# WPI-MMR/gym_solo

Hardware: AMD Instinct MI355X
Metric: env-steps/s (whole node), 4096 Solo8 envs/GPU, 1/2/4/8 MI355X (higher is better)
Workload: dtype f64

## Files before the change

gym_solo_amd/csrc/solo_step_kernel.h:

```cpp
#pragma once

#include "solo_kernel_params.h"
#include "solo_outputs.h"

#if defined(SOLO_STAMPS) && defined(SOLO_STAMPS_LIGHT)
#define SOLO_STAMP(B, i)                                                                          \
  do {                                                                                            \
    if (((i) == 0 || (i) == 14) && solo::lane_id() == 0)                                          \
      (B).stamps[(size_t)(B).stamp_row * 32 + (i)] = __builtin_amdgcn_s_memrealtime();         \
  } while (0)
#elif defined(SOLO_STAMPS)
#ifdef SOLO_STAMPS_EPILOGUE
#define SOLO_STAMP_ON(i) ((i) == 0 || (i) >= 13)
#define SOLO_STAMP_E(B, i) SOLO_STAMP_AT(B, i)
#else
#define SOLO_STAMP_ON(i) true
#endif
#define SOLO_STAMP(B, i) do { if (SOLO_STAMP_ON(i)) SOLO_STAMP_AT(B, i); } while (0)
#define SOLO_STAMP_AT(B, i)                                                                       \
  do {                                                                                            \
    if (solo::lane_id() == 0) {                                                                   \
      const unsigned long long t_ = __builtin_amdgcn_s_memtime();                                 \
      (B).stamps[(size_t)(B).stamp_row * 32 + (i)] = t_;                                            \
      (B).acc[(i)] += t_ - (B).acc[16];                                                           \
      (B).acc[16] = t_;                                                                           \
    }                                                                                             \
  } while (0)
#else
#define SOLO_STAMP(B, i) do {} while (0)
#endif
#ifndef SOLO_STAMP_E
#define SOLO_STAMP_E(B, i) do {} while (0)
#endif

#ifndef SOLO_PGS_SWEEP_HOOK
#define SOLO_PGS_SWEEP_HOOK(it, pend, lam, v) do {} while (0)
#endif

namespace solo {

template <typename T> struct V3 { T x, y, z; };
template <typename T> __device__ __forceinline__ V3<T> operator+(V3<T> a, V3<T> b) { return {a.x + b.x, a.y + b.y, a.z + b.z}; }
template <typename T> __device__ __forceinline__ V3<T> operator-(V3<T> a, V3<T> b) { return {a.x - b.x, a.y - b.y, a.z - b.z}; }
template <typename T> __device__ __forceinline__ V3<T> operator*(T s, V3<T> a) { return {s * a.x, s * a.y, s * a.z}; }
template <typename T> __device__ __forceinline__ T dot(V3<T> a, V3<T> b) { return a.x * b.x + a.y * b.y + a.z * b.z; }
template <typename T> __device__ __forceinline__ V3<T> cross(V3<T> a, V3<T> b) {
  return {a.y * b.z - a.z * b.y, a.z * b.x - a.x * b.z, a.x * b.y - a.y * b.x};
}
template <typename T> __device__ __forceinline__ V3<T> roty(T c, T s, V3<T> v) {
  return {c * v.x + s * v.z, v.y, c * v.z - s * v.x};
}
template <typename T> __device__ __forceinline__ V3<T> ycross(V3<T> r) { return {r.z, T(0), -r.x}; }
template <typename T> __device__ __forceinline__ V3<T> symmul(const T* I, V3<T> v) {
  return {I[0] * v.x + I[3] * v.y + I[4] * v.z, I[3] * v.x + I[1] * v.y + I[5] * v.z,
          I[4] * v.x + I[5] * v.y + I[2] * v.z};
}
template <typename T> __device__ __forceinline__ void rot_inertia_y(T c, T s, const T* I, T* o) {
  const T cc = c * c, ss = s * s, cs = c * s;
  o[0] = cc * I[0] + T(2) * cs * I[4] + ss * I[2];
  o[1] = I[1];
  o[2] = ss * I[0] - T(2) * cs * I[4] + cc * I[2];
  o[3] = c * I[3] + s * I[5];
  o[4] = cs * (I[2] - I[0]) + (cc - ss) * I[4];
  o[5] = c * I[5] - s * I[3];
}
template <typename T> __device__ __forceinline__ T sum_over_group16(T x) { return wave_sum_group16(x); }
template <typename T> __device__ __forceinline__ V3<T> select(bool p, V3<T> a, V3<T> b) { return {p ? a.x : b.x, p ? a.y : b.y, p ? a.z : b.z}; }
template <typename T> __device__ __forceinline__ T both_halves(T x) { return x + wave_other_half16(x); }
template <typename T> __device__ __forceinline__ V3<T> both_halves(V3<T> v) { return {both_halves(v.x), both_halves(v.y), both_halves(v.z)}; }
template <typename T> __device__ __forceinline__ T from_lower(T x) { return wave_from_lower_half16(x); }
template <typename T> __device__ __forceinline__ V3<T> from_lower(V3<T> v) { return {from_lower(v.x), from_lower(v.y), from_lower(v.z)}; }


}
namespace solo {
#ifndef SOLO_PRIO_SWEEPS_F64
#define SOLO_PRIO_SWEEPS_F64 12
#endif
#ifndef SOLO_QUEUE_SPINS
#define SOLO_QUEUE_SPINS (1 << 22)
#endif
#ifndef SOLO_PRIO_BY_ROWS
#define SOLO_PRIO_BY_ROWS 1
#endif
#ifndef SOLO_PRIO_ROWS_1
#define SOLO_PRIO_ROWS_1 11
#define SOLO_PRIO_ROWS_2 17
#define SOLO_PRIO_ROWS_3 23
#endif
__device__ __forceinline__ int priority_by_rows(int rows) { return rows > SOLO_PRIO_ROWS_3 ? 3 : (rows > SOLO_PRIO_ROWS_2 ? 2 : (rows > SOLO_PRIO_ROWS_1 ? 1 : 0)); }
template <typename T> constexpr int kPrioSweeps = sizeof(T) == 4 ? 8 : SOLO_PRIO_SWEEPS_F64;
#ifndef SOLO_F64_WAVES
#define SOLO_F64_WAVES 4
#endif
template <typename T> constexpr int kRowBlockReals = sizeof(T) == 4 ? 64 * 8 + 64 * 8 : (SOLO_F64_WAVES >= 4 ? 800 : 896);
#ifndef SOLO_W4_PIPELINED_BUILD
#define SOLO_W4_PIPELINED_BUILD 0
#endif
#ifndef SOLO_W4_HYBRID_BUILD
#define SOLO_W4_HYBRID_BUILD 1
#endif
constexpr int kLegSlots = 26;

template <typename T> struct RowView {
  int type, body;
  const T* geo;
};
template <typename T> struct StepTables {
  const LegConst<T>* legc;
  const int32_t* rowtype;
  const T (*rowgeo)[4];
  __device__ __forceinline__ RowView<T> row(int lane) const {
    const int tb = rowtype[lane];
    return {tb & 15, (tb >> 4) & 15, rowgeo[(tb >> 8) & 255]};
  }
};

constexpr unsigned long long kPhaseLanes[3] = {0xc003c003c003c003ull,
                                               0x0924092409240924ull,
                                               0x36d836d836d836d8ull};

template <typename T, bool kResid, bool kFromLds>
__device__ __forceinline__ int pgs_solve_cpp(const ColumnBank<T>& A, T& v, T& lamv, T& cand, T& dl, unsigned long long& pend, T& lo, T& hi,
                                             T tol_rel, int lane, T mu, bool is_tan1, bool is_tangent, unsigned long long ph0,
                                             unsigned long long ph1, unsigned long long ph2, int iters, T diag, T resid_thr, int& n_changed) {
  using R = Real<T>;
  int it = 0;
#pragma unroll 1
  for (; it < iters && pend != 0ull; ++it) {
    const T lam_sweep_start = lamv;
    bool normals_moved = false;
#pragma unroll
    for (int phase = 0; phase < 3; ++phase) {
      const unsigned long long phase_lanes = phase == 0 ? ph0 : (phase == 1 ? ph1 : ph2);
      if (phase == 2 && normals_moved) {
        T n1, n2;
        if constexpr (ColumnBank<T>::kCompact) { n1 = wave_slot_below<1>(lamv); n2 = wave_slot_below<2>(lamv); }
        else { n1 = wave_lane_below<1>(lamv); n2 = wave_lane_below<2>(lamv); }
        const T lim = mu * (is_tan1 ? n1 : n2);
        lo = is_tangent ? -lim : lo;
        hi = is_tangent ? lim : hi;
        cand = R::clamp(v, lo, hi);
        dl = cand - lamv;
        pend = wave_ballot(R::abs(dl) > R::abs(lamv) * tol_rel);
      }
      if ((pend & phase_lanes) == 0ull) continue;
      if (phase == 1) normals_moved = true;
#pragma unroll
      for (int bank = 0; bank < (kFromLds ? 1 : ColumnBank<T>::kBanks); ++bank) {
        unsigned long long window = kFromLds ? phase_lanes : (phase_lanes & ColumnBank<T>::bank_lanes(bank));
#pragma unroll 1
        while ((pend & window) != 0ull) {
          const int r = __builtin_ctzll(pend & window);
          window &= ~((2ull << r) - 1ull);
          const T col = kFromLds ? A.column(r) : A.get(bank, r);
          const T delta = wave_readlane(dl, r);
          v = R::fma(col, delta, v);
          lamv = (lane == r) ? cand : lamv;
          cand = R::clamp(v, lo, hi);
          dl = cand - lamv;
          pend = wave_ballot(R::abs(dl) > R::abs(lamv) * tol_rel);
          ++n_changed;
        }
      }
    }
    SOLO_PGS_SWEEP_HOOK(it, pend, lamv, v);
    const T dvel = (lamv - lam_sweep_start) * diag;
    if (kResid && wave_ballot(dvel * dvel > resid_thr) == 0ull) { ++it; break; }
  }
  return it;
}

template <typename T, bool kResid, bool kPipelinedBuild, bool kCtl = false, bool kContact = false, typename FetchTarget>
__device__ __forceinline__ T physics_solve(const StepConst<T>& C, const KBuffers<T>& B, const StepTables<T>& tabs,
                                           const T* s_state, T my_target, FetchTarget&& fetch_target, T* s_rowvec, T (*s_hext)[8], unsigned char* s_rowleg,
                                           T* s_keep, T (*s_leg)[kLegSlots], const T* s_math, T mu, T mass_scale, int lane, int& row_at, bool& target_bad,
                                           int& prio_sweeps, int& prio_steps, int& prio_rot, T warm_in = T(0), bool warm_on = false,
                                           const CtlConst<T>* ctl = nullptr, T* s_cnrm = nullptr) {
  constexpr bool kCompact = ColumnBank<T>::kCompact;
  constexpr int kRS = ColumnBank<T>::kRowStride;
  using R = Real<T>;
  int leg = lane >> 4, k = lane & 15;
  const LegConst<T>* Lp = &tabs.legc[leg];
#define L (*Lp)

  const bool lower = (k & 8) != 0;
  const T bm = lower ? T(1) : T(0);
  const T q1 = s_state[SOLO_S_Q + 2 * leg], q2 = s_state[SOLO_S_Q + 2 * leg + 1];
  const T qd1 = s_state[SOLO_S_QD + 2 * leg], qd2 = s_state[SOLO_S_QD + 2 * leg + 1];
  T sinb, cosb;
  R::sincos(lower ? q1 + q2 : q1, &sinb, &cosb, s_math);
  const T s1 = wave_from_upper_half16(sinb), c1 = wave_from_upper_half16(cosb);
  const T s12 = wave_from_lower_half16(sinb), c12 = wave_from_lower_half16(cosb);
  const V3<T> o1 = {L.hip[0], L.hip[1], L.hip[2]};
  const V3<T> o2 = o1 + roty(c1, s1, V3<T>{L.knee[0], L.knee[1], L.knee[2]});
  const V3<T> ob = select(lower, o2, o1);
  const T* body = L.link[lower ? 1 : 0];
  const T mB = body[0];
  const V3<T> c = ob + roty(cosb, sinb, V3<T>{body[1], body[2], body[3]});
  T I[6];
  rot_inertia_y(cosb, sinb, body + 4, I);

  SOLO_STAMP(B, 2);
  const V3<T> r1 = c - o1, r2 = c - o2;
  const V3<T> t1 = ycross(r1), t2 = ycross(r2);
  const V3<T> Iy = {I[3], I[1], I[5]};
  const V3<T> f1 = both_halves(mB * t1);
  const V3<T> n1 = both_halves(Iy + mB * cross(c, t1));
  const T P11 = both_halves(mB * dot(t1, t1) + I[1]);
  const V3<T> f2 = from_lower(mB * t2);
  const V3<T> n2 = from_lower(Iy + mB * cross(c, t2));
  const T P12 = from_lower(mB * dot(t1, t2) + I[1]);
  const T P22 = from_lower(mB * dot(t2, t2) + I[1]);
  const T iL11 = R::rsqrt(P11);
  const T L21 = P12 * iL11;
  const T iL22 = R::rsqrt(P22 - L21 * L21);
  T W1[6] = {n1.x * iL11, n1.y * iL11, n1.z * iL11, f1.x * iL11, f1.y * iL11, f1.z * iL11};
  const T F2[6] = {n2.x, n2.y, n2.z, f2.x, f2.y, f2.z};
  T W2[6], K1[6], K2[6];
#pragma unroll
  for (int i = 0; i < 6; ++i) {
    W2[i] = (F2[i] - L21 * W1[i]) * iL22;
    K2[i] = W2[i] * iL22;
    K1[i] = (W1[i] - L21 * K2[i]) * iL11;
  }
  constexpr bool kPark = sizeof(T) == 8;
  if constexpr (kPark) {
    if (k == 0) {
#pragma unroll
      for (int i = 0; i < 6; ++i) { s_leg[leg][i] = K1[i]; s_leg[leg][6 + i] = K2[i]; }
      s_leg[leg][12] = iL11; s_leg[leg][13] = L21; s_leg[leg][14] = iL22;
      s_leg[leg][17] = q1; s_leg[leg][18] = q2;
      s_leg[leg][19] = c1; s_leg[leg][20] = s1; s_leg[leg][21] = c12; s_leg[leg][22] = s12;
    }
  }
  const T mleg = L.link[0][0] + L.link[1][0];
  const V3<T> mc = both_halves(mB * c);
  T IO[6];
  IO[0] = both_halves(I[0] + mB * (c.y * c.y + c.z * c.z));
  IO[1] = both_halves(I[1] + mB * (c.x * c.x + c.z * c.z));
  IO[2] = both_halves(I[2] + mB * (c.x * c.x + c.y * c.y));
  IO[3] = both_halves(I[3] - mB * c.x * c.y);
  IO[4] = both_halves(I[4] - mB * c.x * c.z);
  IO[5] = both_halves(I[5] - mB * c.y * c.z);
  if constexpr (kPark) {
    if (k == 0) {
      T* mine = s_rowvec + leg * 32;
#pragma unroll
      for (int i = 0; i < 6; ++i) { mine[i] = IO[i]; mine[17 + i] = W1[i]; mine[24 + i] = W2[i]; }
      mine[6] = mc.x; mine[7] = mc.y; mine[8] = mc.z; mine[9] = mleg; mine[10] = T(0);
    }
    my_target = fetch_target(wave_fresh_lane());
  }

  SOLO_STAMP(B, 3);
  const T qx = s_state[SOLO_S_QUAT], qy = s_state[SOLO_S_QUAT + 1], qz = s_state[SOLO_S_QUAT + 2], qw = s_state[SOLO_S_QUAT + 3];
  const T r00 = T(1) - T(2) * (qy * qy + qz * qz), r01 = T(2) * (qx * qy - qw * qz), r02 = T(2) * (qx * qz + qw * qy);
  const T r10 = T(2) * (qx * qy + qw * qz), r11 = T(1) - T(2) * (qx * qx + qz * qz), r12 = T(2) * (qy * qz - qw * qx);
  const T r20 = T(2) * (qx * qz - qw * qy), r21 = T(2) * (qy * qz + qw * qx), r22 = T(1) - T(2) * (qx * qx + qy * qy);
  const V3<T> ww = {s_state[SOLO_S_ANGVEL], s_state[SOLO_S_ANGVEL + 1], s_state[SOLO_S_ANGVEL + 2]};
  const V3<T> vw = {s_state[SOLO_S_LINVEL], s_state[SOLO_S_LINVEL + 1], s_state[SOLO_S_LINVEL + 2]};
  const V3<T> gw = {C.gravity[0], C.gravity[1], C.gravity[2]};
  const V3<T> om = {r00 * ww.x + r10 * ww.y + r20 * ww.z, r01 * ww.x + r11 * ww.y + r21 * ww.z, r02 * ww.x + r12 * ww.y + r22 * ww.z};
  const V3<T> vb = {r00 * vw.x + r10 * vw.y + r20 * vw.z, r01 * vw.x + r11 * vw.y + r21 * vw.z, r02 * vw.x + r12 * vw.y + r22 * vw.z};
  const V3<T> gb = {r00 * gw.x + r10 * gw.y + r20 * gw.z, r01 * gw.x + r11 * gw.y + r21 * gw.z, r02 * gw.x + r12 * gw.y + r22 * gw.z};
  const V3<T> nb = {r20, r21, r22};

  const V3<T> wU = {om.x, om.y + qd1, om.z};
  const V3<T> wB = {om.x, wU.y + bm * qd2, om.z};
  const V3<T> aU = {-qd1 * om.z, T(0), qd1 * om.x};
  const V3<T> a = {aU.x - (bm * qd2) * wU.z, T(0), aU.z + (bm * qd2) * wU.x};
  const T om2 = dot(om, om), wU2 = dot(wU, wU), wB2 = dot(wB, wB);
  const V3<T> a_o1 = dot(om, o1) * om - om2 * o1;
  const V3<T> d12 = o2 - o1;
  const V3<T> a_o2 = a_o1 + cross(aU, d12) + (dot(wU, d12) * wU - wU2 * d12);
  const V3<T> r = c - ob;
  const V3<T> a_c = select(lower, a_o2, a_o1) + cross(a, r) + (dot(wB, r) * wB - wB2 * r);
  const V3<T> v_c = vb + cross(om, c) + qd1 * t1 + (bm * qd2) * t2;
  const T kl = C.lin_damp, ka = C.ang_damp;
  const T dB = kl * (T(1) + R::sqrt(dot(v_c, v_c)));
  const T eB = ka * (T(1) + R::sqrt(wB2));
  const V3<T> F = mB * (a_c - gb + dB * v_c);
  const V3<T> Iw = symmul(I, wB);
  const V3<T> N = symmul(I, a) + cross(wB, Iw) + eB * Iw;
  const T h1 = both_halves(N.y + (r1.z * F.x - r1.x * F.z));
  const T h2 = from_lower(N.y + (r2.z * F.x - r2.x * F.z));
  const V3<T> Fleg = both_halves(F);
  const V3<T> Nleg = both_halves(N + cross(c, F));
  const T e1 = h1 * iL11, e2 = (h2 - L21 * e1) * iL22;
  const T y2 = e2 * iL22, y1 = (e1 - L21 * y2) * iL11;
  if constexpr (kPark) { if (k == 0) { s_leg[leg][23] = y1; s_leg[leg][24] = y2; } }

  SOLO_STAMP(B, 4);
  T S[6][6];
  S[0][0] = IO[0]; S[1][0] = IO[3]; S[1][1] = IO[1]; S[2][0] = IO[4]; S[2][1] = IO[5]; S[2][2] = IO[2];
  S[3][0] = T(0);  S[3][1] = mc.z;  S[3][2] = -mc.y;
  S[4][0] = -mc.z; S[4][1] = T(0);  S[4][2] = mc.x;
  S[5][0] = mc.y;  S[5][1] = -mc.x; S[5][2] = T(0);
  S[3][3] = mleg; S[4][3] = T(0); S[4][4] = mleg; S[5][3] = T(0); S[5][4] = T(0); S[5][5] = mleg;
  T rhs[6] = {-Nleg.x, -Nleg.y, -Nleg.z, -Fleg.x, -Fleg.y, -Fleg.z};
  if constexpr (kPark) {
    T* part = s_rowvec;
    T* tot = part + 4 * 32;
    if (k == 0) {
      T* mine = part + leg * 32;
#pragma unroll
      for (int i = 0; i < 6; ++i) mine[11 + i] = rhs[i];
      mine[23] = -e1; mine[30] = -e2;
    }
    wave_sync();
    const int ls = wave_fresh_lane();
    lane = ls; leg = ls >> 4; k = ls & 15;
    if (ls < 27) {
      const int tb = tabs.rowtype[ls] >> 16;
      const int bi = tb & 31, ii = (tb >> 6) & 7, jj = (tb >> 9) & 7;
      T t[4];
#pragma unroll
      for (int l2 = 0; l2 < 4; ++l2) {
        const T* p = part + 32 * l2;
        const T b = (tb & 32) ? -p[bi] : p[bi];
        t[l2] = R::fma(-p[24 + ii], p[24 + jj], R::fma(-p[17 + ii], p[17 + jj], b));
      }
      tot[ls] = (t[0] + t[1]) + (t[2] + t[3]);
    }
    wave_sync();
    int o = 0;
#pragma unroll
    for (int i = 0; i < 6; ++i) {
#pragma unroll
      for (int j = 0; j <= i; ++j) S[i][j] = tot[o++];
      rhs[i] = tot[21 + i];
    }
  } else {
    T* part = s_rowvec;
    T* tot = part + 4 * 28;
    if (k == 0) {
      T* mine = part + leg * 28;
      int o = 0;
#pragma unroll
      for (int i = 0; i < 6; ++i) {
#pragma unroll
        for (int j = 0; j <= i; ++j) mine[o++] = S[i][j] - W1[i] * W1[j] - W2[i] * W2[j];
        mine[21 + i] = rhs[i] + W1[i] * e1 + W2[i] * e2;
      }
    }
    wave_sync();
    if (lane < 27) tot[lane] = (part[lane] + part[28 + lane]) + (part[56 + lane] + part[84 + lane]);
    wave_sync();
    int o = 0;
#pragma unroll
    for (int i = 0; i < 6; ++i) {
#pragma unroll
      for (int j = 0; j <= i; ++j) S[i][j] = tot[o++];
      rhs[i] = tot[21 + i];
    }
  }
  if constexpr (sizeof(T) == 8) mass_scale = s_keep[28];
  const T dt = C.dt;
  {
    const T m0 = C.base_mass * mass_scale;
    T I0[6];
#pragma unroll
    for (int i = 0; i < 6; ++i) I0[i] = C.base_I[i] * mass_scale;
    S[0][0] += I0[0]; S[1][0] += I0[3]; S[1][1] += I0[1]; S[2][0] += I0[4]; S[2][1] += I0[5]; S[2][2] += I0[2];
    S[3][3] += m0; S[4][4] += m0; S[5][5] += m0;
    const V3<T> Iw = symmul(I0, om);
    const V3<T> N0 = cross(om, Iw) + (ka * (T(1) + R::sqrt(om2))) * Iw;
    const V3<T> F0 = m0 * ((kl * (T(1) + R::sqrt(dot(vb, vb)))) * vb - gb);
    rhs[0] -= N0.x; rhs[1] -= N0.y; rhs[2] -= N0.z;
    rhs[3] -= F0.x; rhs[4] -= F0.y; rhs[5] -= F0.z;
  }
  SOLO_STAMP(B, 5);
  T iC[6];
#pragma unroll
  for (int j = 0; j < 6; ++j) {
    T d = S[j][j];
#pragma unroll
    for (int m = 0; m < j; ++m) d -= S[j][m] * S[j][m];
    iC[j] = R::rsqrt(d);
#pragma unroll
    for (int i = j + 1; i < 6; ++i) {
      T s = S[i][j];
#pragma unroll
      for (int m = 0; m < j; ++m) s -= S[i][m] * S[j][m];
      S[i][j] = s * iC[j];
    }
  }
  T xb[6];
#pragma unroll
  for (int i = 0; i < 6; ++i) {
    T s = rhs[i];
#pragma unroll
    for (int m = 0; m < i; ++m) s -= S[i][m] * xb[m];
    xb[i] = s * iC[i];
  }
#pragma unroll
  for (int i = 5; i >= 0; --i) {
    T s = xb[i];
#pragma unroll
    for (int m = i + 1; m < 6; ++m) s -= S[m][i] * xb[m];
    xb[i] = s * iC[i];
  }
  T kx1 = T(0), kx2 = T(0);
#pragma unroll
  for (int i = 0; i < 6; ++i) {
    if constexpr (kPark) { kx1 += s_leg[leg][i] * xb[i]; kx2 += s_leg[leg][6 + i] * xb[i]; }
    else { kx1 += K1[i] * xb[i]; kx2 += K2[i] * xb[i]; }
  }
  const T ub[6] = {om.x + dt * xb[0], om.y + dt * xb[1], om.z + dt * xb[2],
             vb.x + dt * xb[3], vb.y + dt * xb[4], vb.z + dt * xb[5]};
  T us1, us2;
  if constexpr (kPark) {
    us1 = s_state[SOLO_S_QD + 2 * leg] + dt * (-s_leg[leg][23] - kx1);
    us2 = s_state[SOLO_S_QD + 2 * leg + 1] + dt * (-s_leg[leg][24] - kx2);
  } else {
    us1 = qd1 + dt * (-y1 - kx1);
    us2 = qd2 + dt * (-y2 - kx2);
  }

  if (lane == 0) {
    int o = 0;
#pragma unroll
    for (int i = 1; i < 6; ++i)
#pragma unroll
      for (int j = 0; j < i; ++j) s_keep[o++] = S[i][j];
#pragma unroll
    for (int i = 0; i < 6; ++i) { s_keep[15 + i] = iC[i]; s_keep[21 + i] = ub[i]; }
  }
  if (k == 0) {
    if constexpr (!kPark) {
#pragma unroll
      for (int i = 0; i < 6; ++i) { s_leg[leg][i] = K1[i]; s_leg[leg][6 + i] = K2[i]; }
      s_leg[leg][12] = iL11; s_leg[leg][13] = L21; s_leg[leg][14] = iL22;
      s_leg[leg][17] = q1; s_leg[leg][18] = q2;
    }
    s_leg[leg][15] = us1; s_leg[leg][16] = us2;
  }
  wave_sync();

  SOLO_STAMP(B, 6);
  T m00 = r00, m01 = r01, m02 = r02, m10 = r10, m11 = r11, m12 = r12;
  V3<T> nbr = nb, p1 = o1, p2 = o2;
  T ck1 = c1, sk1 = s1, ck12 = c12, sk12 = s12, qa1 = q1, qa2 = q2;
  if constexpr (kPark) {
    lane = wave_fresh_lane(); leg = lane >> 4; k = lane & 15;
    Lp = &tabs.legc[leg];
    const T ux = s_state[SOLO_S_QUAT], uy = s_state[SOLO_S_QUAT + 1], uz = s_state[SOLO_S_QUAT + 2], uw = s_state[SOLO_S_QUAT + 3];
    m00 = T(1) - T(2) * (uy * uy + uz * uz); m01 = T(2) * (ux * uy - uw * uz); m02 = T(2) * (ux * uz + uw * uy);
    m10 = T(2) * (ux * uy + uw * uz); m11 = T(1) - T(2) * (ux * ux + uz * uz); m12 = T(2) * (uy * uz - uw * ux);
    nbr = V3<T>{T(2) * (ux * uz - uw * uy), T(2) * (uy * uz + uw * ux), T(1) - T(2) * (ux * ux + uy * uy)};
    qa1 = s_leg[leg][17]; qa2 = s_leg[leg][18];
    ck1 = s_leg[leg][19]; sk1 = s_leg[leg][20]; ck12 = s_leg[leg][21]; sk12 = s_leg[leg][22];
    p1 = V3<T>{L.hip[0], L.hip[1], L.hip[2]};
    p2 = p1 + roty(ck1, sk1, V3<T>{L.knee[0], L.knee[1], L.knee[2]});
  }
  const RowView<T> rc = tabs.row(lane);
  const int type = rc.type;
  const bool is_motor = type == ROW_MOTOR, is_contact = type >= ROW_NORMAL && type <= ROW_TAN2, is_limit = type == ROW_LIMIT;
  V3<T> cb = {rc.geo[0], rc.geo[1], rc.geo[2]};
  const T radius = rc.geo[3];
  if (rc.body == BODY_UPPER) cb = p1 + roty(ck1, sk1, cb);
  else if (rc.body == BODY_LOWER) cb = p2 + roty(ck12, sk12, cb);
  T dist;
  V3<T> nloc = nbr;
  V3<T> d = nbr;
  if (B.terrain == nullptr) {
    dist = s_state[SOLO_S_POS + 2] + dot(nbr, cb) - radius;
    if (type == ROW_TAN1) d = V3<T>{m00, m01, m02};
    if (type == ROW_TAN2) d = V3<T>{m10, m11, m12};
  } else {
    const T cwx = s_state[SOLO_S_POS] + m00 * cb.x + m01 * cb.y + m02 * cb.z;
    const T cwy = s_state[SOLO_S_POS + 1] + m10 * cb.x + m11 * cb.y + m12 * cb.z;
    const T cwz = s_state[SOLO_S_POS + 2] + nbr.x * cb.x + nbr.y * cb.y + nbr.z * cb.z;
    const T gu = (cwx - C.terr_ox) * C.terr_inv_cell, gv = (cwy - C.terr_oy) * C.terr_inv_cell;
    int gi = (int)R::floor(gu), gj = (int)R::floor(gv);
    gi = gi < 0 ? 0 : (gi > C.terr_nx - 2 ? C.terr_nx - 2 : gi);
    gj = gj < 0 ? 0 : (gj > C.terr_ny - 2 ? C.terr_ny - 2 : gj);
    const T fu = R::clamp(gu - T(gi), T(0), T(1)), fv = R::clamp(gv - T(gj), T(0), T(1));
    const T* H = B.terrain + (size_t)gj * C.terr_nx + gi;
    const T h00 = H[0], h10 = H[1], h01 = H[C.terr_nx], h11 = H[C.terr_nx + 1];
    const T hh0 = (T(1) - fu) * (T(1) - fv) * h00 + fu * (T(1) - fv) * h10 + (T(1) - fu) * fv * h01 + fu * fv * h11;
    const T hx = ((T(1) - fv) * (h10 - h00) + fv * (h11 - h01)) * C.terr_inv_cell;
    const T hy = ((T(1) - fu) * (h01 - h00) + fu * (h11 - h10)) * C.terr_inv_cell;
    const T inv = R::rsqrt(hx * hx + hy * hy + T(1));
    const V3<T> nw = {-hx * inv, -hy * inv, inv};
    if constexpr (kContact) {
      if (type == ROW_NORMAL) {
        T* cn = s_cnrm + 3 * (4 * leg + (k - 2) / 3);
        cn[0] = nw.x; cn[1] = nw.y; cn[2] = nw.z;
      }
    }
    const T itn = R::rsqrt(T(1) - nw.x * nw.x);
    const V3<T> t1w = {(T(1) - nw.x * nw.x) * itn, -nw.x * nw.y * itn, -nw.x * nw.z * itn};
    const V3<T> t2w = cross(nw, t1w);
    dist = (cwz - hh0) * nw.z - radius;
    V3<T> dw = nw;
    if (type == ROW_TAN1) dw = t1w;
    if (type == ROW_TAN2) dw = t2w;
    nloc = V3<T>{m00 * nw.x + m10 * nw.y + nbr.x * nw.z, m01 * nw.x + m11 * nw.y + nbr.y * nw.z, m02 * nw.x + m12 * nw.y + nbr.z * nw.z};
    d = V3<T>{m00 * dw.x + m10 * dw.y + nbr.x * dw.z, m01 * dw.x + m11 * dw.y + nbr.y * dw.z, m02 * dw.x + m12 * dw.y + nbr.z * dw.z};
  }
  const int ldof = k & 1;
  const T qlim = ldof == 0 ? qa1 : qa2;
  const T c_lo = qlim - L.limit[ldof][0], c_hi = L.limit[ldof][1] - qlim;
  const T lim_dir = c_lo < c_hi ? T(1) : T(-1), lim_dist = c_lo < c_hi ? c_lo : c_hi;
  const bool live = is_motor || (is_contact && dist < C.margin) || (is_limit && lim_dist < C.limit_margin);
  const V3<T> x = cb - radius * nloc;
  T jb[6] = {T(0), T(0), T(0), T(0), T(0), T(0)};
  T jl1 = T(0), jl2 = T(0), bias = T(0);
  T ctl_imp = T(0);
  if (is_contact) {
    const V3<T> xd = cross(x, d);
    jb[0] = xd.x; jb[1] = xd.y; jb[2] = xd.z; jb[3] = d.x; jb[4] = d.y; jb[5] = d.z;
    if (rc.body != BODY_BASE) jl1 = dot(d, ycross(x - p1));
    if (rc.body == BODY_LOWER) jl2 = dot(d, ycross(x - p2));
    if (type == ROW_NORMAL) bias = (dist > T(0)) ? -dist * C.inv_dt : -C.erp_over_dt * dist;
  } else if (is_motor) {
    jl1 = (k == 0) ? T(1) : T(0);
    jl2 = (k == 1) ? T(1) : T(0);
// ... 467 lines not shown
```

gym_solo_amd/csrc/solo_wave_ops.h:

```cpp
#pragma once

#include <hip/hip_runtime.h>

namespace solo {

__device__ __forceinline__ int lane_id() { return threadIdx.x; }
__device__ __forceinline__ int block_id() { return blockIdx.x; }

__device__ __forceinline__ void wave_sync() { __syncthreads(); }
__device__ __forceinline__ void wave_fence_global() {
  __builtin_amdgcn_fence(__ATOMIC_RELEASE, "workgroup");
  __builtin_amdgcn_fence(__ATOMIC_ACQUIRE, "workgroup");
}
template <typename P> __device__ __forceinline__ P* wave_opaque(P* p) {
  asm volatile("" : "+s"(p));
  return p;
}
__device__ __forceinline__ unsigned long long wave_opaque_bits(unsigned long long x) {
  asm volatile("" : "+s"(x));
  return x;
}
__device__ __forceinline__ int wave_opaque_lane(int lane) {
  asm volatile("" : "+v"(lane));
  return lane;
}
__device__ __forceinline__ int wave_fresh_lane() {
  int lane;
  asm volatile("v_mbcnt_lo_u32_b32 %0, -1, 0\n\tv_mbcnt_hi_u32_b32 %0, -1, %0" : "=v"(lane));
  return lane;
}
__device__ __forceinline__ int wave_readlane_int(int x, int lane) { return __builtin_amdgcn_readlane(x, lane); }
__device__ __forceinline__ int wave_uniform(int x) { return __builtin_amdgcn_readfirstlane(x); }

__device__ __forceinline__ float wave_readlane(float x, int lane) {
  return __int_as_float(__builtin_amdgcn_readlane(__float_as_int(x), lane));
}
__device__ __forceinline__ double wave_readlane(double x, int lane) {
  const long long b = __double_as_longlong(x);
  const int lo = __builtin_amdgcn_readlane((int)(b & 0xffffffffll), lane);
  const int hi = __builtin_amdgcn_readlane((int)(b >> 32), lane);
  return __longlong_as_double(((long long)hi << 32) | (unsigned int)lo);
}
__device__ __forceinline__ float wave_sum_legs(float x) {
  auto a = __builtin_amdgcn_permlane16_swap(__float_as_uint(x), __float_as_uint(x), false, false);
  const float s = __uint_as_float(a[0]) + __uint_as_float(a[1]);
  auto b = __builtin_amdgcn_permlane32_swap(__float_as_uint(s), __float_as_uint(s), false, false);
  return __uint_as_float(b[0]) + __uint_as_float(b[1]);
}
__device__ __forceinline__ double wave_sum_legs(double x) {
  unsigned lo = (unsigned)(__double_as_longlong(x) & 0xffffffffll), hi = (unsigned)(__double_as_longlong(x) >> 32);
  auto a = __builtin_amdgcn_permlane16_swap(lo, lo, false, false);
  auto b = __builtin_amdgcn_permlane16_swap(hi, hi, false, false);
  const double s = __longlong_as_double(((long long)a[0] & 0xffffffffll) | ((long long)b[0] << 32)) +
                   __longlong_as_double(((long long)a[1] & 0xffffffffll) | ((long long)b[1] << 32));
  lo = (unsigned)(__double_as_longlong(s) & 0xffffffffll); hi = (unsigned)(__double_as_longlong(s) >> 32);
  auto c = __builtin_amdgcn_permlane32_swap(lo, lo, false, false);
  auto d = __builtin_amdgcn_permlane32_swap(hi, hi, false, false);
  return __longlong_as_double(((long long)c[0] & 0xffffffffll) | ((long long)d[0] << 32)) +
         __longlong_as_double(((long long)c[1] & 0xffffffffll) | ((long long)d[1] << 32));
}
template <int CTRL> __device__ __forceinline__ float dpp_mov(float x) {
  return __int_as_float(__builtin_amdgcn_update_dpp(0, __float_as_int(x), CTRL, 0xf, 0xf, true));
}
template <int CTRL> __device__ __forceinline__ double dpp_mov(double x) {
  const long long b = __double_as_longlong(x);
  const int lo = __builtin_amdgcn_update_dpp(0, (int)(b & 0xffffffffll), CTRL, 0xf, 0xf, false);
  const int hi = __builtin_amdgcn_update_dpp(0, (int)(b >> 32), CTRL, 0xf, 0xf, false);
  return __longlong_as_double(((long long)hi << 32) | (unsigned int)lo);
}
template <typename T> __device__ __forceinline__ T wave_other_half16(T x) { return dpp_mov<0x128>(x); }
template <int BANKS> __device__ __forceinline__ float dpp_half_bcast(float x) {
  return __int_as_float(__builtin_amdgcn_update_dpp(__float_as_int(x), __float_as_int(x), 0x128, 0xf, BANKS, false));
}
template <int BANKS> __device__ __forceinline__ double dpp_half_bcast(double x) {
  const long long b = __double_as_longlong(x);
  const int lo = __builtin_amdgcn_update_dpp((int)(b & 0xffffffffll), (int)(b & 0xffffffffll), 0x128, 0xf, BANKS, false);
  const int hi = __builtin_amdgcn_update_dpp((int)(b >> 32), (int)(b >> 32), 0x128, 0xf, BANKS, false);
  return __longlong_as_double(((long long)hi << 32) | (unsigned int)lo);
}
template <typename T> __device__ __forceinline__ T wave_from_lower_half16(T x) { return dpp_half_bcast<0x3>(x); }
template <typename T> __device__ __forceinline__ T wave_from_upper_half16(T x) { return dpp_half_bcast<0xc>(x); }
template <int N, typename T> __device__ __forceinline__ T wave_lane_below(T x) { return dpp_mov<0x110 + N>(x); }
template <int N, typename T> __device__ __forceinline__ T wave_slot_below(T x) {
#pragma unroll
  for (int i = 0; i < N; ++i) x = dpp_mov<0x138>(x);
  return x;
}
__device__ __forceinline__ int wave_count_below(unsigned long long mask) {
  return (int)__builtin_amdgcn_mbcnt_hi((unsigned)(mask >> 32), __builtin_amdgcn_mbcnt_lo((unsigned)mask, 0u));
}
__device__ __forceinline__ int wave_push_int(int x, int dst) { return __builtin_amdgcn_ds_permute(dst << 2, x); }
__device__ __forceinline__ float wave_push(float x, int dst) { return __int_as_float(__builtin_amdgcn_ds_permute(dst << 2, __float_as_int(x))); }
__device__ __forceinline__ double wave_push(double x, int dst) {
  const long long b = __double_as_longlong(x);
  const int lo = __builtin_amdgcn_ds_permute(dst << 2, (int)(b & 0xffffffffll));
  const int hi = __builtin_amdgcn_ds_permute(dst << 2, (int)(b >> 32));
  return __longlong_as_double(((long long)hi << 32) | (unsigned int)lo);
}
__device__ __forceinline__ float wave_pull(float x, int src) { return __int_as_float(__builtin_amdgcn_ds_bpermute(src << 2, __float_as_int(x))); }
__device__ __forceinline__ double wave_pull(double x, int src) {
  const long long b = __double_as_longlong(x);
  const int lo = __builtin_amdgcn_ds_bpermute(src << 2, (int)(b & 0xffffffffll));
  const int hi = __builtin_amdgcn_ds_bpermute(src << 2, (int)(b >> 32));
  return __longlong_as_double(((long long)hi << 32) | (unsigned int)lo);
}
template <typename T> __device__ __forceinline__ T wave_sum_group16(T x) {
  x += dpp_mov<0x128>(x);
  x += dpp_mov<0x124>(x);
  x += dpp_mov<0x122>(x);
  x += dpp_mov<0x121>(x);
  return x;
}
__device__ __forceinline__ float wave_sum_all(float x) {
  x = wave_sum_group16(x);
  asm("s_nop 1\n\tv_add_f32_dpp %0, %0, %0 row_bcast:15 row_mask:0xa bank_mask:0xf\n\t"
      "s_nop 1\n\tv_add_f32_dpp %0, %0, %0 row_bcast:31 row_mask:0xc bank_mask:0xf" : "+v"(x));
  return wave_readlane(x, 63);
}
__device__ __forceinline__ double wave_sum_all(double x) { return wave_sum_legs(wave_sum_group16(x)); }
__device__ __forceinline__ unsigned long long wave_ballot(bool p) { return __ballot(p); }

__device__ __forceinline__ void wave_reduce_rows(float (&z)[6], float (&y)[2]) {
#define SOLO_DPP_STAGE8(CTRL)                                                                      \
  "v_add_f32_dpp %0, %0, %0 " CTRL " row_mask:0xf bank_mask:0xf\n\t"                                \
  "v_add_f32_dpp %1, %1, %1 " CTRL " row_mask:0xf bank_mask:0xf\n\t"                                \
  "v_add_f32_dpp %2, %2, %2 " CTRL " row_mask:0xf bank_mask:0xf\n\t"                                \
  "v_add_f32_dpp %3, %3, %3 " CTRL " row_mask:0xf bank_mask:0xf\n\t"                                \
  "v_add_f32_dpp %4, %4, %4 " CTRL " row_mask:0xf bank_mask:0xf\n\t"                                \
  "v_add_f32_dpp %5, %5, %5 " CTRL " row_mask:0xf bank_mask:0xf\n\t"                                \
  "v_add_f32_dpp %6, %6, %6 " CTRL " row_mask:0xf bank_mask:0xf\n\t"                                \
  "v_add_f32_dpp %7, %7, %7 " CTRL " row_mask:0xf bank_mask:0xf\n\t"
#define SOLO_DPP_STAGE6(CTRL, MASK)                                                                \
  "v_add_f32_dpp %0, %0, %0 " CTRL " row_mask:" MASK " bank_mask:0xf\n\t"                           \
  "v_add_f32_dpp %1, %1, %1 " CTRL " row_mask:" MASK " bank_mask:0xf\n\t"                           \
  "v_add_f32_dpp %2, %2, %2 " CTRL " row_mask:" MASK " bank_mask:0xf\n\t"                           \
  "v_add_f32_dpp %3, %3, %3 " CTRL " row_mask:" MASK " bank_mask:0xf\n\t"                           \
  "v_add_f32_dpp %4, %4, %4 " CTRL " row_mask:" MASK " bank_mask:0xf\n\t"                           \
  "v_add_f32_dpp %5, %5, %5 " CTRL " row_mask:" MASK " bank_mask:0xf\n\t"
  asm("s_nop 1\n\t"
      SOLO_DPP_STAGE8("row_ror:8") SOLO_DPP_STAGE8("row_ror:4") SOLO_DPP_STAGE8("row_ror:2") SOLO_DPP_STAGE8("row_ror:1")
      SOLO_DPP_STAGE6("row_bcast:15", "0xa") SOLO_DPP_STAGE6("row_bcast:31", "0xc")
      : "+v"(z[0]), "+v"(z[1]), "+v"(z[2]), "+v"(z[3]), "+v"(z[4]), "+v"(z[5]), "+v"(y[0]), "+v"(y[1]));
#undef SOLO_DPP_STAGE8
#undef SOLO_DPP_STAGE6
#pragma unroll
  for (int i = 0; i < 6; ++i) z[i] = wave_readlane(z[i], 63);
}
__device__ __forceinline__ void wave_reduce_rows(double (&z)[6], double (&y)[2]) {
#pragma unroll
  for (int i = 0; i < 6; ++i) z[i] = wave_sum_all(z[i]);
  y[0] = wave_sum_group16(y[0]);
  y[1] = wave_sum_group16(y[1]);
}
constexpr int kReduceScratch = 64 * 9;
template <int N> __device__ __forceinline__ double dpp_row_bcast(double x) {
  const long long b = __double_as_longlong(x);
  const int lo = __builtin_amdgcn_update_dpp(0, (int)(b & 0xffffffffll), 0x150 + N, 0xf, 0xf, false);
  const int hi = __builtin_amdgcn_update_dpp(0, (int)(b >> 32), 0x150 + N, 0xf, 0xf, false);
  return __longlong_as_double(((long long)hi << 32) | (unsigned int)lo);
}
__device__ __forceinline__ void wave_reduce_rows_lds(double (&z)[6], double (&y)[2], double* scratch, int lane) {
  double* const mine = scratch + lane * 9;
#pragma unroll
  for (int i = 0; i < 6; ++i) mine[i] = z[i];
// ... 332 lines not shown
```

Baseline: 190.9 million.

## Compute f64 leg dynamics on half-wave with 8-lane groups per leg

For f64, leg dynamics now use 8 lanes per leg instead of 16, so all four legs fit in the lower 32 lanes and the upper half of the wave is masked off. New 8-lane DPP helpers (row_half_mirror-style controls with bank masks) replace the 16-lane half-broadcast and reduction primitives. The later base solve is also restricted to lanes below 32, using a per-lane leg index. The goal is to cut redundant f64 VALU work per wave. The risk is that wave-wide instruction cost on masked lanes may not drop, and the extra divergence and control flow can add overhead.

```diff
diff --git a/gym_solo_amd/csrc/solo_step_kernel.h b/gym_solo_amd/csrc/solo_step_kernel.h
--- a/gym_solo_amd/csrc/solo_step_kernel.h
+++ b/gym_solo_amd/csrc/solo_step_kernel.h
@@ -37,7 +37,22 @@
 #define SOLO_PGS_SWEEP_HOOK(it, pend, lam, v) do {} while (0)
 #endif
 
+#ifndef SOLO_HALF_WAVE_DYNAMICS
+#define SOLO_HALF_WAVE_DYNAMICS 1
+#endif
+
 namespace solo {
+
+#ifndef __HIPCC__
+template <typename T> inline T wave_other_half8(T x) { return wave_readlane(x, lane_id() ^ 4); }
+template <typename T> inline T wave_from_lower_half8(T x) { const T o = wave_readlane(x, lane_id() ^ 4); return (lane_id() & 4) ? x : o; }
+template <typename T> inline T wave_from_upper_half8(T x) { const T o = wave_readlane(x, lane_id() ^ 4); return (lane_id() & 4) ? o : x; }
+constexpr bool kHalfWaveMaskCrossLane = false;
+#else
+constexpr bool kHalfWaveMaskCrossLane = true;
+#endif
+template <typename T> constexpr bool kHalfWaveBase = sizeof(T) == 8 && SOLO_HALF_WAVE_DYNAMICS != 0;
+template <typename T> constexpr bool kHalfWaveDyn = sizeof(T) == 8 && SOLO_HALF_WAVE_DYNAMICS == 1;
 
 template <typename T> struct V3 { T x, y, z; };
 template <typename T> __device__ __forceinline__ V3<T> operator+(V3<T> a, V3<T> b) { return {a.x + b.x, a.y + b.y, a.z + b.z}; }
@@ -66,10 +81,11 @@
 }
 template <typename T> __device__ __forceinline__ T sum_over_group16(T x) { return wave_sum_group16(x); }
 template <typename T> __device__ __forceinline__ V3<T> select(bool p, V3<T> a, V3<T> b) { return {p ? a.x : b.x, p ? a.y : b.y, p ? a.z : b.z}; }
-template <typename T> __device__ __forceinline__ T both_halves(T x) { return x + wave_other_half16(x); }
-template <typename T> __device__ __forceinline__ V3<T> both_halves(V3<T> v) { return {both_halves(v.x), both_halves(v.y), both_halves(v.z)}; }
-template <typename T> __device__ __forceinline__ T from_lower(T x) { return wave_from_lower_half16(x); }
-template <typename T> __device__ __forceinline__ V3<T> from_lower(V3<T> v) { return {from_lower(v.x), from_lower(v.y), from_lower(v.z)}; }
+template <bool k8 = false, typename T> __device__ __forceinline__ T both_halves(T x) { if constexpr (k8) return x + wave_other_half8(x); else return x + wave_other_half16(x); }
+template <bool k8 = false, typename T> __device__ __forceinline__ V3<T> both_halves(V3<T> v) { return {both_halves<k8>(v.x), both_halves<k8>(v.y), both_halves<k8>(v.z)}; }
+template <bool k8 = false, typename T> __device__ __forceinline__ T from_lower(T x) { if constexpr (k8) return wave_from_lower_half8(x); else return wave_from_lower_half16(x); }
+template <bool k8 = false, typename T> __device__ __forceinline__ V3<T> from_lower(V3<T> v) { return {from_lower<k8>(v.x), from_lower<k8>(v.y), from_lower<k8>(v.z)}; }
+template <bool k8 = false, typename T> __device__ __forceinline__ T from_upper(T x) { if constexpr (k8) return wave_from_upper_half8(x); else return wave_from_upper_half16(x); }
 
 
 }
@@ -180,20 +196,29 @@
   constexpr bool kCompact = ColumnBank<T>::kCompact;
   constexpr int kRS = ColumnBank<T>::kRowStride;
   using R = Real<T>;
-  int leg = lane >> 4, k = lane & 15;
+  constexpr bool kPark = sizeof(T) == 8;
+  constexpr bool kH = kHalfWaveDyn<T>;
+  int leg = kH ? (lane & 31) >> 3 : lane >> 4, k = kH ? lane & 7 : lane & 15;
   const LegConst<T>* Lp = &tabs.legc[leg];
 #define L (*Lp)
-
-  const bool lower = (k & 8) != 0;
+  T K1[6], K2[6], W1[6], W2[6], iL11, L21, iL22, q1, q2, qd1, qd2, s1, c1, s12, c12, e1, e2, y1, y2;
+  T r00, r01, r02, r10, r11, r12, om2, kl, ka;
+  V3<T> o1, o2, om, vb, gb, nb;
+  T S[6][6];
+  T rhs[6];
+  const auto post = [&] { return k == 0 && (!kH || lane < 32); };
+  if (!kH || !kHalfWaveMaskCrossLane || lane < 32) {
+
+  const bool lower = (k & (kH ? 4 : 8)) != 0;
   const T bm = lower ? T(1) : T(0);
-  const T q1 = s_state[SOLO_S_Q + 2 * leg], q2 = s_state[SOLO_S_Q + 2 * leg + 1];
-  const T qd1 = s_state[SOLO_S_QD + 2 * leg], qd2 = s_state[SOLO_S_QD + 2 * leg + 1];
+  q1 = s_state[SOLO_S_Q + 2 * leg]; q2 = s_state[SOLO_S_Q + 2 * leg + 1];
+  qd1 = s_state[SOLO_S_QD + 2 * leg]; qd2 = s_state[SOLO_S_QD + 2 * leg + 1];
   T sinb, cosb;
   R::sincos(lower ? q1 + q2 : q1, &sinb, &cosb, s_math);
-  const T s1 = wave_from_upper_half16(sinb), c1 = wave_from_upper_half16(cosb);
-  const T s12 = wave_from_lower_half16(sinb), c12 = wave_from_lower_half16(cosb);
-  const V3<T> o1 = {L.hip[0], L.hip[1], L.hip[2]};
-  const V3<T> o2 = o1 + roty(c1, s1, V3<T>{L.knee[0], L.knee[1], L.knee[2]});
+  s1 = from_upper<kH>(sinb); c1 = from_upper<kH>(cosb);
+  s12 = from_lower<kH>(sinb); c12 = from_lower<kH>(cosb);
+  o1 = V3<T>{L.hip[0], L.hip[1], L.hip[2]};
+  o2 = o1 + roty(c1, s1, V3<T>{L.knee[0], L.knee[1], L.knee[2]});
   const V3<T> ob = select(lower, o2, o1);
   const T* body = L.link[lower ? 1 : 0];
   const T mB = body[0];
@@ -205,28 +230,26 @@
   const V3<T> r1 = c - o1, r2 = c - o2;
   const V3<T> t1 = ycross(r1), t2 = ycross(r2);
   const V3<T> Iy = {I[3], I[1], I[5]};
-  const V3<T> f1 = both_halves(mB * t1);
-  const V3<T> n1 = both_halves(Iy + mB * cross(c, t1));
-  const T P11 = both_halves(mB * dot(t1, t1) + I[1]);
-  const V3<T> f2 = from_lower(mB * t2);
-  const V3<T> n2 = from_lower(Iy + mB * cross(c, t2));
-  const T P12 = from_lower(mB * dot(t1, t2) + I[1]);
-  const T P22 = from_lower(mB * dot(t2, t2) + I[1]);
-  const T iL11 = R::rsqrt(P11);
-  const T L21 = P12 * iL11;
-  const T iL22 = R::rsqrt(P22 - L21 * L21);
-  T W1[6] = {n1.x * iL11, n1.y * iL11, n1.z * iL11, f1.x * iL11, f1.y * iL11, f1.z * iL11};
+  const V3<T> f1 = both_halves<kH>(mB * t1);
+  const V3<T> n1 = both_halves<kH>(Iy + mB * cross(c, t1));
+  const T P11 = both_halves<kH>(mB * dot(t1, t1) + I[1]);
+  const V3<T> f2 = from_lower<kH>(mB * t2);
+  const V3<T> n2 = from_lower<kH>(Iy + mB * cross(c, t2));
+  const T P12 = from_lower<kH>(mB * dot(t1, t2) + I[1]);
+  const T P22 = from_lower<kH>(mB * dot(t2, t2) + I[1]);
+  iL11 = R::rsqrt(P11);
+  L21 = P12 * iL11;
+  iL22 = R::rsqrt(P22 - L21 * L21);
+  W1[0] = n1.x * iL11; W1[1] = n1.y * iL11; W1[2] = n1.z * iL11; W1[3] = f1.x * iL11; W1[4] = f1.y * iL11; W1[5] = f1.z * iL11;
   const T F2[6] = {n2.x, n2.y, n2.z, f2.x, f2.y, f2.z};
-  T W2[6], K1[6], K2[6];
 #pragma unroll
   for (int i = 0; i < 6; ++i) {
     W2[i] = (F2[i] - L21 * W1[i]) * iL22;
     K2[i] = W2[i] * iL22;
     K1[i] = (W1[i] - L21 * K2[i]) * iL11;
   }
-  constexpr bool kPark = sizeof(T) == 8;
   if constexpr (kPark) {
-    if (k == 0) {
+    if (post()) {
 #pragma unroll
       for (int i = 0; i < 6; ++i) { s_leg[leg][i] = K1[i]; s_leg[leg][6 + i] = K2[i]; }
       s_leg[leg][12] = iL11; s_leg[leg][13] = L21; s_leg[leg][14] = iL22;
@@ -235,79 +258,85 @@
     }
   }
   const T mleg = L.link[0][0] + L.link[1][0];
-  const V3<T> mc = both_halves(mB * c);
+  const V3<T> mc = both_halves<kH>(mB * c);
   T IO[6];
-  IO[0] = both_halves(I[0] + mB * (c.y * c.y + c.z * c.z));
-  IO[1] = both_halves(I[1] + mB * (c.x * c.x + c.z * c.z));
-  IO[2] = both_halves(I[2] + mB * (c.x * c.x + c.y * c.y));
-  IO[3] = both_halves(I[3] - mB * c.x * c.y);
-  IO[4] = both_halves(I[4] - mB * c.x * c.z);
-  IO[5] = both_halves(I[5] - mB * c.y * c.z);
+  IO[0] = both_halves<kH>(I[0] + mB * (c.y * c.y + c.z * c.z));
+  IO[1] = both_halves<kH>(I[1] + mB * (c.x * c.x + c.z * c.z));
+  IO[2] = both_halves<kH>(I[2] + mB * (c.x * c.x + c.y * c.y));
+  IO[3] = both_halves<kH>(I[3] - mB * c.x * c.y);
+  IO[4] = both_halves<kH>(I[4] - mB * c.x * c.z);
+  IO[5] = both_halves<kH>(I[5] - mB * c.y * c.z);
   if constexpr (kPark) {
-    if (k == 0) {
+    if (post()) {
       T* mine = s_rowvec + leg * 32;
 #pragma unroll
       for (int i = 0; i < 6; ++i) { mine[i] = IO[i]; mine[17 + i] = W1[i]; mine[24 + i] = W2[i]; }
       mine[6] = mc.x; mine[7] = mc.y; mine[8] = mc.z; mine[9] = mleg; mine[10] = T(0);
     }
-    my_target = fetch_target(wave_fresh_lane());
+    if constexpr (!kH) my_target = fetch_target(wave_fresh_lane());
   }
 
   SOLO_STAMP(B, 3);
   const T qx = s_state[SOLO_S_QUAT], qy = s_state[SOLO_S_QUAT + 1], qz = s_state[SOLO_S_QUAT + 2], qw = s_state[SOLO_S_QUAT + 3];
-  const T r00 = T(1) - T(2) * (qy * qy + qz * qz), r01 = T(2) * (qx * qy - qw * qz), r02 = T(2) * (qx * qz + qw * qy);
-  const T r10 = T(2) * (qx * qy + qw * qz), r11 = T(1) - T(2) * (qx * qx + qz * qz), r12 = T(2) * (qy * qz - qw * qx);
+  r00 = T(1) - T(2) * (qy * qy + qz * qz); r01 = T(2) * (qx * qy - qw * qz); r02 = T(2) * (qx * qz + qw * qy);
+  r10 = T(2) * (qx * qy + qw * qz); r11 = T(1) - T(2) * (qx * qx + qz * qz); r12 = T(2) * (qy * qz - qw * qx);
   const T r20 = T(2) * (qx * qz - qw * qy), r21 = T(2) * (qy * qz + qw * qx), r22 = T(1) - T(2) * (qx * qx + qy * qy);
   const V3<T> ww = {s_state[SOLO_S_ANGVEL], s_state[SOLO_S_ANGVEL + 1], s_state[SOLO_S_ANGVEL + 2]};
   const V3<T> vw = {s_state[SOLO_S_LINVEL], s_state[SOLO_S_LINVEL + 1], s_state[SOLO_S_LINVEL + 2]};
   const V3<T> gw = {C.gravity[0], C.gravity[1], C.gravity[2]};
-  const V3<T> om = {r00 * ww.x + r10 * ww.y + r20 * ww.z, r01 * ww.x + r11 * ww.y + r21 * ww.z, r02 * ww.x + r12 * ww.y + r22 * ww.z};
-  const V3<T> vb = {r00 * vw.x + r10 * vw.y + r20 * vw.z, r01 * vw.x + r11 * vw.y + r21 * vw.z, r02 * vw.x + r12 * vw.y + r22 * vw.z};
-  const V3<T> gb = {r00 * gw.x + r10 * gw.y + r20 * gw.z, r01 * gw.x + r11 * gw.y + r21 * gw.z, r02 * gw.x + r12 * gw.y + r22 * gw.z};
-  const V3<T> nb = {r20, r21, r22};
+  om = V3<T>{r00 * ww.x + r10 * ww.y + r20 * ww.z, r01 * ww.x + r11 * ww.y + r21 * ww.z, r02 * ww.x + r12 * ww.y + r22 * ww.z};
+  vb = V3<T>{r00 * vw.x + r10 * vw.y + r20 * vw.z, r01 * vw.x + r11 * vw.y + r21 * vw.z, r02 * vw.x + r12 * vw.y + r22 * vw.z};
+  gb = V3<T>{r00 * gw.x + r10 * gw.y + r20 * gw.z, r01 * gw.x + r11 * gw.y + r21 * gw.z, r02 * gw.x + r12 * gw.y + r22 * gw.z};
+  nb = V3<T>{r20, r21, r22};
 
   const V3<T> wU = {om.x, om.y + qd1, om.z};
   const V3<T> wB = {om.x, wU.y + bm * qd2, om.z};
   const V3<T> aU = {-qd1 * om.z, T(0), qd1 * om.x};
   const V3<T> a = {aU.x - (bm * qd2) * wU.z, T(0), aU.z + (bm * qd2) * wU.x};
-  const T om2 = dot(om, om), wU2 = dot(wU, wU), wB2 = dot(wB, wB);
+  om2 = dot(om, om);
+  const T wU2 = dot(wU, wU), wB2 = dot(wB, wB);
   const V3<T> a_o1 = dot(om, o1) * om - om2 * o1;
   const V3<T> d12 = o2 - o1;
   const V3<T> a_o2 = a_o1 + cross(aU, d12) + (dot(wU, d12) * wU - wU2 * d12);
   const V3<T> r = c - ob;
   const V3<T> a_c = select(lower, a_o2, a_o1) + cross(a, r) + (dot(wB, r) * wB - wB2 * r);
   const V3<T> v_c = vb + cross(om, c) + qd1 * t1 + (bm * qd2) * t2;
-  const T kl = C.lin_damp, ka = C.ang_damp;
+  kl = C.lin_damp; ka = C.ang_damp;
   const T dB = kl * (T(1) + R::sqrt(dot(v_c, v_c)));
   const T eB = ka * (T(1) + R::sqrt(wB2));
   const V3<T> F = mB * (a_c - gb + dB * v_c);
   const V3<T> Iw = symmul(I, wB);
   const V3<T> N = symmul(I, a) + cross(wB, Iw) + eB * Iw;
-  const T h1 = both_halves(N.y + (r1.z * F.x - r1.x * F.z));
-  const T h2 = from_lower(N.y + (r2.z * F.x - r2.x * F.z));
-  const V3<T> Fleg = both_halves(F);
-  const V3<T> Nleg = both_halves(N + cross(c, F));
-  const T e1 = h1 * iL11, e2 = (h2 - L21 * e1) * iL22;
-  const T y2 = e2 * iL22, y1 = (e1 - L21 * y2) * iL11;
-  if constexpr (kPark) { if (k == 0) { s_leg[leg][23] = y1; s_leg[leg][24] = y2; } }
+  const T h1 = both_halves<kH>(N.y + (r1.z * F.x - r1.x * F.z));
+  const T h2 = from_lower<kH>(N.y + (r2.z * F.x - r2.x * F.z));
+  const V3<T> Fleg = both_halves<kH>(F);
+  const V3<T> Nleg = both_halves<kH>(N + cross(c, F));
+  e1 = h1 * iL11; e2 = (h2 - L21 * e1) * iL22;
+  y2 = e2 * iL22; y1 = (e1 - L21 * y2) * iL11;
+  if constexpr (kPark) { if (post()) { s_leg[leg][23] = y1; s_leg[leg][24] = y2; } }
 
   SOLO_STAMP(B, 4);
-  T S[6][6];
   S[0][0] = IO[0]; S[1][0] = IO[3]; S[1][1] = IO[1]; S[2][0] = IO[4]; S[2][1] = IO[5]; S[2][2] = IO[2];
   S[3][0] = T(0);  S[3][1] = mc.z;  S[3][2] = -mc.y;
   S[4][0] = -mc.z; S[4][1] = T(0);  S[4][2] = mc.x;
   S[5][0] = mc.y;  S[5][1] = -mc.x; S[5][2] = T(0);
   S[3][3] = mleg; S[4][3] = T(0); S[4][4] = mleg; S[5][3] = T(0); S[5][4] = T(0); S[5][5] = mleg;
-  T rhs[6] = {-Nleg.x, -Nleg.y, -Nleg.z, -Fleg.x, -Fleg.y, -Fleg.z};
+  rhs[0] = -Nleg.x; rhs[1] = -Nleg.y; rhs[2] = -Nleg.z; rhs[3] = -Fleg.x; rhs[4] = -Fleg.y; rhs[5] = -Fleg.z;
   if constexpr (kPark) {
     T* part = s_rowvec;
     T* tot = part + 4 * 32;
-    if (k == 0) {
+    if (post()) {
       T* mine = part + leg * 32;
 #pragma unroll
       for (int i = 0; i < 6; ++i) mine[11 + i] = rhs[i];
       mine[23] = -e1; mine[30] = -e2;
     }
+  }
+  }
+  if constexpr (kPark) {
+    T* part = s_rowvec;
+    T* tot = part + 4 * 32;
+    if constexpr (kH) my_target = fetch_target(wave_fresh_lane());
     wave_sync();
     const int ls = wave_fresh_lane();
     lane = ls; leg = ls >> 4; k = ls & 15;
@@ -324,13 +353,6 @@
       tot[ls] = (t[0] + t[1]) + (t[2] + t[3]);
     }
     wave_sync();
-    int o = 0;
-#pragma unroll
-    for (int i = 0; i < 6; ++i) {
-#pragma unroll
-      for (int j = 0; j <= i; ++j) S[i][j] = tot[o++];
-      rhs[i] = tot[21 + i];
-    }
   } else {
     T* part = s_rowvec;
     T* tot = part + 4 * 28;
@@ -347,6 +369,13 @@
     wave_sync();
     if (lane < 27) tot[lane] = (part[lane] + part[28 + lane]) + (part[56 + lane] + part[84 + lane]);
     wave_sync();
+  }
+  constexpr bool kHB = kHalfWaveBase<T>;
+  const int bleg = kHB ? (lane & 3) : leg;
+  const auto bpost = [&] { return kHB ? lane < 4 : k == 0; };
+  if (!kHB || lane < 32) {
+  {
+    const T* tot = s_rowvec + 4 * (kPark ? 32 : 28);
     int o = 0;
 #pragma unroll
     for (int i = 0; i < 6; ++i) {
@@ -404,15 +433,15 @@
   T kx1 = T(0), kx2 = T(0);
 #pragma unroll
   for (int i = 0; i < 6; ++i) {
-    if constexpr (kPark) { kx1 += s_leg[leg][i] * xb[i]; kx2 += s_leg[leg][6 + i] * xb[i]; }
+    if constexpr (kPark) { kx1 += s_leg[bleg][i] * xb[i]; kx2 += s_leg[bleg][6 + i] * xb[i]; }
     else { kx1 += K1[i] * xb[i]; kx2 += K2[i] * xb[i]; }
   }
   const T ub[6] = {om.x + dt * xb[0], om.y + dt * xb[1], om.z + dt * xb[2],
              vb.x + dt * xb[3], vb.y + dt * xb[4], vb.z + dt * xb[5]};
   T us1, us2;
   if constexpr (kPark) {
-    us1 = s_state[SOLO_S_QD + 2 * leg] + dt * (-s_leg[leg][23] - kx1);
-    us2 = s_state[SOLO_S_QD + 2 * leg + 1] + dt * (-s_leg[leg][24] - kx2);
+    us1 = s_state[SOLO_S_QD + 2 * bleg] + dt * (-s_leg[bleg][23] - kx1);
+    us2 = s_state[SOLO_S_QD + 2 * bleg + 1] + dt * (-s_leg[bleg][24] - kx2);
   } else {
     us1 = qd1 + dt * (-y1 - kx1);
     us2 = qd2 + dt * (-y2 - kx2);
@@ -427,14 +456,15 @@
 #pragma unroll
     for (int i = 0; i < 6; ++i) { s_keep[15 + i] = iC[i]; s_keep[21 + i] = ub[i]; }
   }
-  if (k == 0) {
+  if (bpost()) {
     if constexpr (!kPark) {
 #pragma unroll
       for (int i = 0; i < 6; ++i) { s_leg[leg][i] = K1[i]; s_leg[leg][6 + i] = K2[i]; }
       s_leg[leg][12] = iL11; s_leg[leg][13] = L21; s_leg[leg][14] = iL22;
       s_leg[leg][17] = q1; s_leg[leg][18] = q2;
     }
-    s_leg[leg][15] = us1; s_leg[leg][16] = us2;
+    s_leg[bleg][15] = us1; s_leg[bleg][16] = us2;
+  }
   }
   wave_sync();
 
diff --git a/gym_solo_amd/csrc/solo_wave_ops.h b/gym_solo_amd/csrc/solo_wave_ops.h
--- a/gym_solo_amd/csrc/solo_wave_ops.h
+++ b/gym_solo_amd/csrc/solo_wave_ops.h
@@ -69,17 +69,20 @@
   return __longlong_as_double(((long long)hi << 32) | (unsigned int)lo);
 }
 template <typename T> __device__ __forceinline__ T wave_other_half16(T x) { return dpp_mov<0x128>(x); }
-template <int BANKS> __device__ __forceinline__ float dpp_half_bcast(float x) {
-  return __int_as_float(__builtin_amdgcn_update_dpp(__float_as_int(x), __float_as_int(x), 0x128, 0xf, BANKS, false));
-}
-template <int BANKS> __device__ __forceinline__ double dpp_half_bcast(double x) {
-  const long long b = __double_as_longlong(x);
-  const int lo = __builtin_amdgcn_update_dpp((int)(b & 0xffffffffll), (int)(b & 0xffffffffll), 0x128, 0xf, BANKS, false);
-  const int hi = __builtin_amdgcn_update_dpp((int)(b >> 32), (int)(b >> 32), 0x128, 0xf, BANKS, false);
+template <int BANKS, int CTRL = 0x128> __device__ __forceinline__ float dpp_half_bcast(float x) {
+  return __int_as_float(__builtin_amdgcn_update_dpp(__float_as_int(x), __float_as_int(x), CTRL, 0xf, BANKS, false));
+}
+template <int BANKS, int CTRL = 0x128> __device__ __forceinline__ double dpp_half_bcast(double x) {
+  const long long b = __double_as_longlong(x);
+  const int lo = __builtin_amdgcn_update_dpp((int)(b & 0xffffffffll), (int)(b & 0xffffffffll), CTRL, 0xf, BANKS, false);
+  const int hi = __builtin_amdgcn_update_dpp((int)(b >> 32), (int)(b >> 32), CTRL, 0xf, BANKS, false);
   return __longlong_as_double(((long long)hi << 32) | (unsigned int)lo);
 }
 template <typename T> __device__ __forceinline__ T wave_from_lower_half16(T x) { return dpp_half_bcast<0x3>(x); }
 template <typename T> __device__ __forceinline__ T wave_from_upper_half16(T x) { return dpp_half_bcast<0xc>(x); }
+template <typename T> __device__ __forceinline__ T wave_other_half8(T x) { return dpp_mov<0x141>(x); }
+template <typename T> __device__ __forceinline__ T wave_from_lower_half8(T x) { return dpp_half_bcast<0x5, 0x141>(x); }
+template <typename T> __device__ __forceinline__ T wave_from_upper_half8(T x) { return dpp_half_bcast<0xa, 0x141>(x); }
 template <int N, typename T> __device__ __forceinline__ T wave_lane_below(T x) { return dpp_mov<0x110 + N>(x); }
 template <int N, typename T> __device__ __forceinline__ T wave_slot_below(T x) {
 #pragma unroll
```

New measurement: 190.9 million (median of 2 runs). Within noise of the previous version (-0.0%).
